# tigarcia/firedancer

Hardware: AMD Instinct MI355X
Metric: ed25519 verifies/sec at 1/8 GPUs; % INT32 VALU roofline; p99 batch latency (higher is better)
Workload: dtype int32

## Files before the change

### firedancer_amd/csrc/fd25519_dsm.h

```cpp
#pragma once
#include "fd25519_ge.h"
#include "fd_ed25519_hip_internal.h"

#define FD_ED25519_SUCCESS 0
#define FD_ED25519_ERR_SIG -1
#define FD_ED25519_ERR_PUBKEY -2
#define FD_ED25519_ERR_MSG -3


struct decoded_pt {
  fe x, y;
  bool fail;
  bool small;
};

FD_DEV void ge_decode(decoded_pt& d, const uint32_t (&s)[8], bool avx_rule) {
  const fe one = {{1, 0, 0, 0, 0, 0, 0, 0, 0, 0}};
  const fe cd = {FE_D}, sqrtm1 = {FE_SQRTM1};
  fe u, v, v3, x, vxx, t;
  fe_frombytes(d.y, s);
  const uint32_t sign = s[7] >> 31;
  fe_sq(u, d.y);
  fe_mul(v, u, cd);
  fe_sub(u, u, one);
// ... 103 lines not shown
  constexpr int W = SH / 32, B = SH % 32;
#pragma unroll
  for (int i = 4; i >= 0; i--) {
    const uint32_t hi = i - W >= 0 ? x[i - W] : 0u;
    const uint32_t lo = i - W - 1 >= 0 ? x[i - W - 1] : 0u;
    out[i] = B ? __builtin_amdgcn_alignbit(hi, lo, 32 - B) : hi;
  }
}

FD_DEV void shl160v(uint32_t (&out)[5], const uint32_t (&x)[5], int s) {
#pragma unroll
  for (int i = 4; i > 0; i--) out[i] = __builtin_amdgcn_alignbit(x[i], x[i - 1], 32 - s);
  out[0] = x[0] << s;
}

template <int BITS>
FD_DEV void recode160(uint32_t (&out)[5], const uint32_t (&x)[5]) {
  constexpr uint32_t M = (1u << BITS) - 1u;
  constexpr int PER = 32 / BITS;
  int carry = 0;
#pragma unroll
  for (int w = 0; w < 5; w++) {
    uint32_t packed = 0;
#pragma unroll
    for (int q = 0; q < PER; q++) {
      int e = (int)((x[w] >> (BITS * q)) & M) + carry;
      carry = (e + (1 << (BITS - 1))) >> BITS;
      e -= carry << BITS;
      packed |= ((uint32_t)e & M) << (BITS * q);
    }
    out[w] = packed;
  }
}

template <int BITS>
FD_DEV uint32_t pop160u(uint32_t (&d)[5]) {
  const uint32_t v = d[4] >> (32 - BITS);
#pragma unroll
  for (int w = 4; w > 0; w--) d[w] = __builtin_amdgcn_alignbit(d[w], d[w - 1], 32 - BITS);
  d[0] <<= BITS;
  return v;
}

template <int BITS>
FD_DEV int pop160(uint32_t (&d)[5]) {
  const int v = ((int32_t)d[4]) >> (32 - BITS);
#pragma unroll
  for (int w = 4; w > 0; w--) d[w] = __builtin_amdgcn_alignbit(d[w], d[w - 1], 32 - BITS);
  d[0] <<= BITS;
  return v;
}


FD_DEV void atab_store(int4* lane_tab, int e, const ge_cached& c) {
  int v[40];
#pragma unroll
  for (int i = 0; i < 10; i++) {
    v[i] = c.YplusX.v[i];
    v[10 + i] = c.YminusX.v[i];
    v[20 + i] = c.Z2.v[i];
    v[30 + i] = c.T2d.v[i];
  }
#pragma unroll
  for (int q = 0; q < 10; q++)
    lane_tab[e * 10 + q] = make_int4(v[4 * q], v[4 * q + 1], v[4 * q + 2], v[4 * q + 3]);
}

FD_DEV void atab_load(ge_cached& c, const int4* lane_tab, int e) {
  int v[40];
#pragma unroll
  for (int q = 0; q < 10; q++) {
    const int4 x = lane_tab[e * 10 + q];
    v[4 * q] = x.x; v[4 * q + 1] = x.y; v[4 * q + 2] = x.z; v[4 * q + 3] = x.w;
  }
#pragma unroll
  for (int i = 0; i < 10; i++) {
    c.YplusX.v[i] = v[i];
    c.YminusX.v[i] = v[10 + i];
    c.Z2.v[i] = v[20 + i];
    c.T2d.v[i] = v[30 + i];
  }
}

FD_DEV void btab_load(ge_precomp& b, const int4* s_btab, int e) {
  int v[32];
  const int4* src = s_btab + e * (FD_ED25519_BTAB_STRIDE / 4);
#pragma unroll
  for (int q = 0; q < 8; q++) {
    const int4 x = src[q];
    v[4 * q] = x.x; v[4 * q + 1] = x.y; v[4 * q + 2] = x.z; v[4 * q + 3] = x.w;
  }
#pragma unroll
  for (int i = 0; i < 10; i++) {
    b.yplusx.v[i] = v[i];
    b.yminusx.v[i] = v[10 + i];
    b.xy2d.v[i] = v[20 + i];
  }
}

FD_DEV void btab16_load(ge_precomp& b, const int4* g_btab, int e) {
  int v[32];
  const int4* src = g_btab + e * (FD_ED25519_BTAB16_STRIDE / 4);
#pragma unroll
  for (int q = 0; q < 8; q++) {
    const int4 x = src[q];
    v[4 * q] = x.x; v[4 * q + 1] = x.y; v[4 * q + 2] = x.z; v[4 * q + 3] = x.w;
  }
#pragma unroll
  for (int i = 0; i < 10; i++) {
    b.yplusx.v[i] = v[i];
    b.yminusx.v[i] = v[10 + i];
    b.xy2d.v[i] = v[20 + i];
  }
}


FD_DEV void ge_scalarmult_base(ge_p2& Q, const uint32_t (&s)[8], const int4* s_btab) {
  uint32_t sd[8];
  recode_radix256(sd, s);
  ge_p3 P;
  ge_p3_0(P);
  ge_p1p1 Rt;
#pragma clang loop unroll(disable)
  for (int j = 31; j >= 0; j--) {
    if (j != 31) {
#pragma clang loop unroll(disable)
      for (int dd = 0; dd < 8; dd++) {
        ge_p2_dbl(Rt, Q);
        if (dd < 7) ge_p1p1_to_p2(Q, Rt);
      }
      ge_p1p1_to_p3(P, Rt);
    }
    const int f = pop_digit<8>(sd);
    ge_precomp b;
    btab_load(b, s_btab, f < 0 ? -f : f);
    ge_precomp_cneg(b, f < 0);
    ge_madd(Rt, P, b);
    ge_p1p1_to_p2(Q, Rt);
  }
}

FD_DEV void ge_encode(uint32_t (&out)[8], const ge_p2& Q) {
  fe zi, x, y;
  fe_invert(zi, Q.Z);
  fe_mul(x, Q.X, zi);
  fe_mul(y, Q.Y, zi);
  uint32_t xb[8];
  fe_tobytes(xb, x);
  fe_tobytes(out, y);
  out[7] |= (xb[0] & 1u) << 31;
}
```

### firedancer_amd/csrc/fd25519_fe.h

```cpp
#pragma once
#include <hip/hip_runtime.h>
#include <stdint.h>

#define FD_DEV __device__ __forceinline__

struct fe { int32_t v[10]; };

#define FE_D      {-10913610, 13857413, -15372611, 6949391, 114729, -8787816, -6275908, -3247719, -18696448, -12055116}
#define FE_D2     {-21827239, -5839606, -30745221, 13898782, 229458, 15978800, -12551817, -6495438, 29715968, 9444199}
#define FE_DINV   {30013526, 3972531, -24787780, 12719051, 2979674, -4599962, -15693209, -3644061, 18959709, -16629253}
#define FE_SQRTM1 {-32595792, -7943725, 9377950, 3500415, 12389472, -272473, -25146209, -2005654, 326686, 11406482}
#define FE_BX     {-14297830, -7645148, 16144683, -16471763, 27570974, -2696100, -26142465, 8378389, 20764389, 8758491}
#define FE_BY     {-26843541, -6710886, 13421773, -13421773, 26843546, 6710886, -13421773, 13421773, -26843546, -6710886}

FD_DEV void fe_set_const(fe& h, const int32_t (&c)[10]) {
#pragma unroll
  for (int i = 0; i < 10; i++) h.v[i] = c[i];
}

FD_DEV void fe_0(fe& h) {
#pragma unroll
  for (int i = 0; i < 10; i++) h.v[i] = 0;
}

// ... 115 lines not shown
      const int k = i + j;
      const int m = (((i & 1) && (j & 1)) ? 2 : 1) * ((k >= 10) ? 19 : 1);
      const int32_t x = (i == j) ? f.v[i] : 2 * f.v[i];
      const int32_t y = m * f.v[j];
      if (i == 0) fe_mad_init(a[k], x, y, k);
      else fe_mad(a[k >= 10 ? k - 10 : k], x, y);
    }
  }
  fe_carry_wide(h, a);
}

FD_DEV void fe_sq2(fe& h, const fe& f) {
  int64_t a[10];
#pragma unroll
  for (int i = 0; i < 10; i++) {
#pragma unroll
    for (int j = i; j < 10; j++) {
      const int k = i + j;
      const int m = (((i & 1) && (j & 1)) ? 2 : 1) * ((k >= 10) ? 19 : 1);
      const int32_t x = (i == j) ? 2 * f.v[i] : 4 * f.v[i];
      const int32_t y = m * f.v[j];
      if (i == 0) fe_mad_init(a[k], x, y, k);
      else fe_mad(a[k >= 10 ? k - 10 : k], x, y);
    }
  }
  fe_carry_wide(h, a);
}

FD_DEV void fe_join_u(int32_t (&u)[10], int64_t c4, int64_t c9) {
  {
    const int64_t t = c4 + (int64_t)(uint32_t)u[5];
    u[5] = (int32_t)t & ((1 << 25) - 1);
    u[6] += (int32_t)(t >> 25);
  }
  {
    const int64_t t = c9 * 19 + (int64_t)(uint32_t)u[0];
    u[0] = (int32_t)t & ((1 << 26) - 1);
    u[1] += (int32_t)(t >> 26);
  }
}

FD_DEV void fe_launder_u(fe& h, int32_t (&u)[10]) {
#pragma unroll
  for (int i = 0; i < 10; i++) {
    asm("" : "+v"(u[i]));
    h.v[i] = u[i];
  }
}

FD_DEV void fe_mul19_u(fe& h, const fe& f, const fe& g, const fe& g19) {
  int32_t u[10];
  int64_t cA = 0, cB = 0;
#pragma unroll
  for (int s = 0; s < 5; s++) {
#pragma unroll
    for (int half = 0; half < 2; half++) {
      const int k = s + 5 * half;
      int64_t acc = half ? cB : cA;
#pragma unroll
      for (int n = 0; n < 10; n++) {
        const int i = n, j = (k - i + 10) % 10;
        const int32_t x = ((i & 1) && (j & 1)) ? 2 * f.v[i] : f.v[i];
        const int32_t y = (i + j >= 10) ? g19.v[j] : g.v[j];
        if (s == 0 && n == 0) acc = (int64_t)x * y;
        else acc += (int64_t)x * y;
#if FE_ASM_MAD
        FE_ACC_BARRIER_U(acc);
#endif
      }
      const int w = (k & 1) ? 25 : 26;
      u[k] = (int32_t)acc & ((1 << w) - 1);
      if (half) cB = acc >> w;
      else cA = acc >> w;
    }
  }
  fe_join_u(u, cA, cB);
  fe_launder_u(h, u);
}

FD_DEV void fe_mul_u(fe& h, const fe& f, const fe& g) {
  fe g19;
  fe_19(g19, g);
  fe_mul19_u(h, f, g, g19);
}

template <int S>
FD_DEV void fe_sqs_u(fe& h, const fe& f) {
  int32_t u[10];
  int64_t cA = 0, cB = 0;
#pragma unroll
  for (int s = 0; s < 5; s++) {
#pragma unroll
    for (int half = 0; half < 2; half++) {
      const int k = s + 5 * half;
      int64_t acc = half ? cB : cA;
      bool first = (s == 0);
#pragma unroll
      for (int i = 0; i < 10; i++) {
#pragma unroll
        for (int j = i; j < 10; j++) {
          if ((i + j) % 10 != k) continue;
          const int m = (((i & 1) && (j & 1)) ? 2 : 1) * ((i + j >= 10) ? 19 : 1);
          const int32_t x = (i == j) ? S * f.v[i] : 2 * S * f.v[i];
          const int32_t y = m * f.v[j];
          if (first) acc = (int64_t)x * y;
          else acc += (int64_t)x * y;
          first = false;
#if FE_ASM_MAD
          FE_ACC_BARRIER_U(acc);
#endif
        }
      }
      const int w = (k & 1) ? 25 : 26;
      u[k] = (int32_t)acc & ((1 << w) - 1);
      if (half) cB = acc >> w;
      else cA = acc >> w;
    }
  }
  fe_join_u(u, cA, cB);
  fe_launder_u(h, u);
}

FD_DEV void fe_sq_u(fe& h, const fe& f) { fe_sqs_u<1>(h, f); }
FD_DEV void fe_sq2_u(fe& h, const fe& f) { fe_sqs_u<2>(h, f); }

FD_DEV void fe_carry(fe& h, const fe& f) {
  int64_t a[10];
#pragma unroll
  for (int i = 0; i < 10; i++) a[i] = (int64_t)f.v[i] + FE_BIAS(i);
  fe_carry_wide(h, a);
}

FD_DEV void fe_frombytes(fe& h, const uint32_t (&w)[8]) {
  const uint32_t m26 = (1u << 26) - 1u, m25 = (1u << 25) - 1u;
  h.v[0] = (int32_t)(w[0] & m26);
  h.v[1] = (int32_t)(__builtin_amdgcn_alignbit(w[1], w[0], 26) & m25);
  h.v[2] = (int32_t)(__builtin_amdgcn_alignbit(w[2], w[1], 19) & m26);
  h.v[3] = (int32_t)(__builtin_amdgcn_alignbit(w[3], w[2], 13) & m25);
  h.v[4] = (int32_t)((w[3] >> 6) & m26);
  h.v[5] = (int32_t)(w[4] & m25);
  h.v[6] = (int32_t)(__builtin_amdgcn_alignbit(w[5], w[4], 25) & m26);
  h.v[7] = (int32_t)(__builtin_amdgcn_alignbit(w[6], w[5], 19) & m25);
  h.v[8] = (int32_t)(__builtin_amdgcn_alignbit(w[7], w[6], 12) & m26);
  h.v[9] = (int32_t)((w[7] >> 6) & m25);
}

FD_DEV void fe_carry(fe& h, const fe& f);
FD_DEV void fe_tobytes(uint32_t (&s)[8], const fe& f) {
  fe g;
  fe_carry(g, f);
  int32_t h[10];
#pragma unroll
  for (int i = 0; i < 10; i++) h[i] = g.v[i];
  int32_t q = (19 * h[9] + (1 << 24)) >> 25;
#pragma unroll
  for (int i = 0; i < 10; i++) q = (h[i] + q) >> ((i & 1) ? 25 : 26);
  h[0] += 19 * q;
  int32_t c;
#pragma unroll
  for (int i = 0; i < 9; i++) {
    const int sh = (i & 1) ? 25 : 26;
    c = h[i] >> sh;
    h[i + 1] += c;
    h[i] -= c * (1 << sh);
  }
  c = h[9] >> 25;
// ... 67 lines not shown
```

### firedancer_amd/csrc/fd25519_ge.h

```cpp
#pragma once
#include "fd25519_fe.h"

struct ge_p2 { fe X, Y, Z; };
struct ge_p3 { fe X, Y, Z, T; };
struct ge_p1p1 { fe X, Y, Z, T; };
struct ge_cached { fe YplusX, YminusX, Z2, T2d; };
struct ge_precomp { fe yplusx, yminusx, xy2d; };

FD_DEV void ge_p3_0(ge_p3& h) {
  fe_0(h.X); fe_1(h.Y); fe_1(h.Z); fe_0(h.T);
}


FD_DEV void ge_p1p1_to_p2(ge_p2& r, const ge_p1p1& p) {
  fe x19, z19;
  fe_19(x19, p.X);
  fe_19(z19, p.Z);
  fe_mul19_u(r.X, p.T, p.X, x19);
  fe_mul19_u(r.Y, p.Y, p.Z, z19);
  fe_mul19_u(r.Z, p.T, p.Z, z19);
}

template <bool UXYT, bool UZ>
FD_DEV void ge_p1p1_to_p3_t(ge_p3& r, const ge_p1p1& p) {
  fe x19, z19;
  fe_19(x19, p.X);
  fe_19(z19, p.Z);
  if (UXYT) {
    fe_mul19_u(r.X, p.T, p.X, x19);
    fe_mul19_u(r.T, p.Y, p.X, x19);
    fe_mul19_u(r.Y, p.Y, p.Z, z19);
  } else {
    fe_mul19(r.X, p.T, p.X, x19);
    fe_mul19(r.T, p.Y, p.X, x19);
    fe_mul19(r.Y, p.Y, p.Z, z19);
  }
  if (UZ) fe_mul19_u(r.Z, p.T, p.Z, z19);
  else fe_mul19(r.Z, p.T, p.Z, z19);
}

FD_DEV void ge_p1p1_to_p3(ge_p3& r, const ge_p1p1& p) { ge_p1p1_to_p3_t<false, false>(r, p); }
FD_DEV void ge_p1p1_to_p3_u(ge_p3& r, const ge_p1p1& p) { ge_p1p1_to_p3_t<true, true>(r, p); }
FD_DEV void ge_p1p1_to_p3_uxyt(ge_p3& r, const ge_p1p1& p) { ge_p1p1_to_p3_t<true, false>(r, p); }

FD_DEV void ge_p2_dbl(ge_p1p1& r, const ge_p2& p) {
  fe xx, yy, b, a, aa;
  fe_sq(xx, p.X);
  fe_sq_u(yy, p.Y);
  fe_sq2_u(b, p.Z);
  fe_sub(a, p.X, p.Y);
  fe_sq_u(aa, a);
  fe_add(r.Y, yy, xx);
  fe_sub(r.Z, yy, xx);
  fe_sub(r.X, r.Y, aa);
  fe_sub(r.T, b, r.Z);
}

FD_DEV void ge_p3_dbl(ge_p1p1& r, const ge_p3& p) {
  ge_p2 q;
  q.X = p.X; q.Y = p.Y; q.Z = p.Z;
  ge_p2_dbl(r, q);
}

#define FE_P_LIMBS {(1 << 26) - 19, (1 << 25) - 1, (1 << 26) - 1, (1 << 25) - 1, (1 << 26) - 1, \
                    (1 << 25) - 1, (1 << 26) - 1, (1 << 25) - 1, (1 << 26) - 1, (1 << 25) - 1}
template <bool UXY = false>
FD_DEV void ge_p3_to_cached(ge_cached& r, const ge_p3& p) {
  const fe d2 = {FE_D2};
  if (UXY) {
    const fe pl = {FE_P_LIMBS};
#pragma unroll
    for (int i = 0; i < 10; i++) r.YplusX.v[i] = p.Y.v[i] + p.X.v[i] - pl.v[i];
  } else {
    fe_add(r.YplusX, p.Y, p.X);
  }
  fe_sub(r.YminusX, p.Y, p.X);
  fe_add(r.Z2, p.Z, p.Z);
  fe_mul_u(r.T2d, p.T, d2);
}

template <bool NT = false>
FD_DEV void ge_add(ge_p1p1& r, const ge_p3& p, const ge_cached& q) {
  fe a, b, c, zz2;
  fe_add(a, p.Y, p.X);
  fe_sub(b, p.Y, p.X);
  fe_mul_u(a, a, q.YplusX);
  fe_mul_u(b, b, q.YminusX);
  fe_mul_u(zz2, p.Z, q.Z2);
  if (NT) fe_mul_u(c, q.T2d, p.T);
  else fe_mul(c, q.T2d, p.T);
  fe_sub(r.X, a, b);
  fe_add(r.Y, a, b);
  if (NT) {
    fe_sub(r.Z, zz2, c);
    fe_add(r.T, zz2, c);
  } else {
    fe_add(r.Z, zz2, c);
    fe_sub(r.T, zz2, c);
  }
}

FD_DEV void ge_madd(ge_p1p1& r, const ge_p3& p, const ge_precomp& q) {
  fe a, b, c, t0;
  fe_add(a, p.Y, p.X);
  fe_sub(b, p.Y, p.X);
  fe_mul_u(a, a, q.yplusx);
  fe_mul_u(b, b, q.yminusx);
  fe_mul(c, q.xy2d, p.T);
  fe_add(t0, p.Z, p.Z);
  fe_sub(r.X, a, b);
  fe_add(r.Y, a, b);
  fe_add(r.Z, t0, c);
  fe_sub(r.T, t0, c);
}

FD_DEV void ge_cached_cneg(ge_cached& q, bool neg) {
  fe t;
#pragma unroll
  for (int i = 0; i < 10; i++) {
    const int32_t a = q.YplusX.v[i], b = q.YminusX.v[i];
    q.YplusX.v[i] = neg ? b : a;
    q.YminusX.v[i] = neg ? a : b;
    t.v[i] = -q.T2d.v[i];
    q.T2d.v[i] = neg ? t.v[i] : q.T2d.v[i];
  }
}

FD_DEV void ge_precomp_cneg(ge_precomp& q, bool neg) {
#pragma unroll
  for (int i = 0; i < 10; i++) {
    const int32_t a = q.yplusx.v[i], b = q.yminusx.v[i];
    q.yplusx.v[i] = neg ? b : a;
    q.yminusx.v[i] = neg ? a : b;
    const int32_t t = q.xy2d.v[i];
    q.xy2d.v[i] = neg ? -t : t;
  }
}
```

### firedancer_amd/csrc/fd_ed25519_kernels.hip

```cpp
#include <hip/hip_runtime.h>
#include "fd25519_dsm.h"
#include "fd25519_ge4.h"
#include "fd25519_sc.h"
#include "fd_sha512_dev.h"
#define FD_HALF_FN __device__ static inline
#define FD_HALF_RCP(y) __builtin_amdgcn_rcp(y)
#define FD_HALF_RCPF(y) __builtin_amdgcn_rcpf(y)
#include "fd25519_half.h"



#define FD_PF_FAIL  1u
#define FD_PF_SMALL 2u
#define FD_HF_DNEG  1u
#define FD_HF_FULL  2u


FD_DEV uint32_t nblk_bucket(uint32_t sz) {
  const uint32_t b = (sz + 208u) >> 7;
  return b < (FD_ED25519_SORT_BUCKETS - 1) ? b : (FD_ED25519_SORT_BUCKETS - 1);
}

#define FD_SORT_PER_THREAD 16
#define FD_SORT_PER_BLOCK (256 * FD_SORT_PER_THREAD)
// ... 92 lines not shown
  uint32_t dig[16];
  if (p.digests) {
    const uint4* dg = reinterpret_cast<const uint4*>(p.digests + 64 * i);
#pragma unroll
    for (int q = 0; q < 4; q++) {
      const uint4 v = dg[q];
      dig[4 * q] = v.x; dig[4 * q + 1] = v.y; dig[4 * q + 2] = v.z; dig[4 * q + 3] = v.w;
    }
  } else {
    const uintptr_t mp = reinterpret_cast<uintptr_t>(p.msgs + p.msg_off[i]);
    sha_msg_src m;
    m.base = reinterpret_cast<const uint32_t*>(mp & ~(uintptr_t)3);
    m.shift = (uint32_t)(mp & 3);
    m.sz = p.msg_sz[i];
    sha512_ram(dig, r, a, m);
  }
  hash_finish(p, j, dig, S);
}

__global__ void __launch_bounds__(256, FD_ED25519_HASH_WAVES_PER_SIMD)
fd_ed25519_hash_kernel(fd_ed25519_verify_params_t p) {
  const uint64_t t = (uint64_t)blockIdx.x * blockDim.x + threadIdx.x;
  if (t >= p.n) return;
  hash_one(p, p.perm ? (uint64_t)p.perm[t] : t);
}

FD_DEV void decode_one(const fd_ed25519_verify_params_t& p, int which , uint64_t j) {
  const uint64_t i = p.base + j;
  uint32_t s[8];
  {
    const uint4* src = which ? reinterpret_cast<const uint4*>(p.sigs + 64 * i)
                             : reinterpret_cast<const uint4*>(p.pubs + 32 * i);
    const uint4 q0 = src[0], q1 = src[1];
    s[0] = q0.x; s[1] = q0.y; s[2] = q0.z; s[3] = q0.w; s[4] = q1.x; s[5] = q1.y; s[6] = q1.z; s[7] = q1.w;
  }
  decoded_pt d;
  ge_decode(d, s, !p.codes_portable);
  int32_t* dst = p.pts + (uint64_t)which * 20 * p.cap + j;
#pragma unroll
  for (int l = 0; l < 10; l++) {
    dst[(uint64_t)l * p.cap] = d.x.v[l];
    dst[(uint64_t)(10 + l) * p.cap] = d.y.v[l];
  }
  p.pflag[(uint64_t)which * p.cap + j] = (uint8_t)((d.fail ? FD_PF_FAIL : 0u) | (d.small ? FD_PF_SMALL : 0u));
}

__global__ void __launch_bounds__(256, FD_ED25519_DECODE_WAVES_PER_SIMD)
fd_ed25519_decode_kernel(fd_ed25519_verify_params_t p) {
  const uint64_t t = (uint64_t)blockIdx.x * blockDim.x + threadIdx.x;
  if (t >= 2 * p.n) return;
  const int which = t >= p.n;
  decode_one(p, which, which ? t - p.n : t);
}

FD_DEV void load_fe(fe& x, const int32_t* src, uint64_t cap) {
#pragma unroll
  for (int l = 0; l < 10; l++) x.v[l] = src[(uint64_t)l * cap];
}

FD_DEV void load_pt(fe& x, fe& y, const fd_ed25519_verify_params_t& p, int which, uint64_t j) {
  const int32_t* src = p.pts + (uint64_t)which * 20 * p.cap + j;
  load_fe(x, src, p.cap);
  load_fe(y, src + 10 * p.cap, p.cap);
}

#define FD_PENDING 1
FD_DEV int precheck(const fd_ed25519_verify_params_t& p, uint64_t j) {
  const uint32_t s_ok = p.sflag[j];
  const uint32_t af = p.pflag[j], rf = p.pflag[p.cap + j];
  if (!s_ok) return FD_ED25519_ERR_SIG;
  if (af & FD_PF_FAIL) return p.codes_portable ? FD_ED25519_ERR_PUBKEY : FD_ED25519_ERR_SIG;
  if (rf & FD_PF_FAIL) return FD_ED25519_ERR_SIG;
  if (af & FD_PF_SMALL) return FD_ED25519_ERR_PUBKEY;
  if (rf & FD_PF_SMALL) return FD_ED25519_ERR_SIG;
  return FD_PENDING;
}

template <bool NT>
FD_DEV void table_store(int4* tab, int e, ge_cached c) {
  if (NT) fe_neg(c.T2d, c.T2d);
  atab_store(tab, e, c);
}

__device__ const int4 fd_ident_cached[10] = {{1, 0, 0, 0}, {0, 0, 0, 0}, {0, 0, 1, 0}, {0, 0, 0, 0}, {0, 0, 0, 0},
                                             {2, 0, 0, 0}, {0, 0, 0, 0}, {0, 0, 0, 0}, {0, 0, 0, 0}, {0, 0, 0, 0}};

template <bool NT>
FD_DEV void table_build(int4* tab, const fe& x, const fe& y, bool negate) {
  ge_p3 P0;
  fe xn;
  fe_neg(xn, x);
  fe_select(P0.X, x, xn, negate);
  P0.Y = y;
  fe_1(P0.Z);
  fe_mul(P0.T, P0.X, y);
  ge_cached c1, c;
  c.YplusX = P0.Z; c.YminusX = P0.Z; fe_add(c.Z2, P0.Z, P0.Z); fe_0(c.T2d);
  atab_store(tab, 0, c);
  ge_p3_to_cached(c1, P0);
  table_store<NT>(tab, 1, c1);
  ge_precomp pre;
  pre.yplusx = c1.YplusX; pre.yminusx = c1.YminusX; pre.xy2d = c1.T2d;
  ge_p3 cur = P0;
  ge_p1p1 sum;
#pragma clang loop unroll(disable)
  for (int e = 2; e <= 8; e++) {
    ge_madd(sum, cur, pre);
    ge_p1p1_to_p3_uxyt(cur, sum);
    ge_p3_to_cached<true>(c, cur);
    table_store<NT>(tab, e, c);
  }
}

FD_DEV void table_add(ge_p1p1& Rt, const ge_p3& P, const int4* tab, int e) {
  ge_cached c;
  atab_load(c, tab, e < 0 ? -e : e);
  ge_cached_cneg(c, e < 0);
  ge_add(Rt, P, c);
}

FD_DEV void btab_add(ge_p1p1& Rt, const ge_p3& P, ge_precomp& b, int f) {
  ge_precomp_cneg(b, f < 0);
  ge_madd(Rt, P, b);
}


FD_DEV bool half_pair_ok(const uint32_t (&k)[8], const uint32_t (&c)[FD_HALF_TW], const uint32_t (&dm)[FD_HALF_TW],
                         int dneg, int dbits) {
  uint32_t x[16];
#pragma unroll
  for (int w = 0; w < 16; w++) x[w] = 0u;
#pragma unroll
  for (int a = 0; a < FD_HALF_TW; a++) {
    uint64_t carry = 0;
#pragma unroll
    for (int b = 0; b < 8; b++) {
      const uint64_t t = (uint64_t)dm[a] * k[b] + x[a + b] + carry;
      x[a + b] = (uint32_t)t;
      carry = t >> 32;
    }
    x[a + 8] = (uint32_t)carry;
  }
  const uint32_t n8l[8] = FD_HALF_N8L;
  uint32_t add[8];
  {
    uint64_t br = 0;
#pragma unroll
    for (int w = 0; w < 8; w++) {
      const uint32_t cv = w < FD_HALF_TW ? c[w] : 0u;
      const uint64_t t = (uint64_t)n8l[w] - cv - br;
      br = (t >> 63) & 1u;
      add[w] = dneg ? cv : (uint32_t)t;
    }
  }
  {
    uint64_t carry = 0;
#pragma unroll
    for (int w = 0; w < 15; w++) {
      const uint64_t t = (uint64_t)x[w] + (w < 8 ? add[w] : 0u) + carry;
      x[w] = (uint32_t)t;
      carry = t >> 32;
    }
  }
  const uint32_t low = x[0] & 7u;
#pragma unroll
  for (int w = 0; w < 15; w++) x[w] = __builtin_amdgcn_alignbit(x[w + 1], x[w], 3);
  x[15] >>= 3;
// ... 79 lines not shown
        const uint64_t t = (uint64_t)l[w] - sp[w] - br;
        br = (t >> 63) & 1u;
        sp[w] = nz ? (uint32_t)t : 0u;
      }
    }
  }
  uint32_t* hs = p.hs + j;
  const uint64_t c = p.cap;
  static_assert(FD_ED25519_BTABW_SHIFT == 144, "s_lo is words 0..3 and the low half of word 4");
#pragma unroll
  for (int w = 0; w < 5; w++) {
    hs[(uint64_t)w * c] = cw[w];
    hs[(uint64_t)(5 + w) * c] = dm[w];
    hs[(uint64_t)(10 + w) * c] = w < 4 ? sp[w] : (sp[4] & 0xffffu);
  }
#pragma unroll
  for (int w = 0; w < 4; w++)
    hs[(uint64_t)(15 + w) * c] = __builtin_amdgcn_alignbit(w + 5 < 8 ? sp[w + 5] : 0u, sp[w + 4], 16);
  p.hflag[j] = (uint8_t)((dneg ? FD_HF_DNEG : 0u) | (ok ? 0u : FD_HF_FULL));
  if (!ok && !p.small) {
    const uint32_t slot = atomicAdd(p.fix_cnt, 1u);
    p.fix_list[slot] = (uint32_t)j;
  }
}

__global__ void __launch_bounds__(256, FD_ED25519_SCALAR_WAVES_PER_SIMD)
fd_ed25519_scalar_kernel(fd_ed25519_verify_params_t p) {
  const uint64_t j = (uint64_t)blockIdx.x * blockDim.x + threadIdx.x;
  if (j >= p.n) return;
  scalar_one(p, j);
}

__global__ void __launch_bounds__(192) fd_ed25519_prep_kernel(fd_ed25519_verify_params_t p) {
  const uint32_t w = threadIdx.x >> 6;
  const uint64_t t = (uint64_t)blockIdx.x * 64u + (threadIdx.x & 63u);
  if (t >= p.n) return;
  if (w == 0) {
    const uint64_t j = p.perm ? (uint64_t)p.perm[t] : t;
    hash_one(p, j);
    scalar_one(p, j);
  } else {
    decode_one(p, (int)w - 1, t);
  }
}


FD_DEV void load_hs(uint32_t (&x)[5], const fd_ed25519_verify_params_t& p, int row, int words, uint64_t j) {
#pragma unroll
  for (int w = 0; w < 5; w++) x[w] = w < words ? p.hs[(uint64_t)(row + w) * p.cap + j] : 0u;
}

template <int BITS>
FD_DEV int wave_windows(const uint32_t (&d)[5]) {
  static_assert(BITS == 2 || BITS == 4, "2-bit or 4-bit windows");
  constexpr int W0 = 132 / BITS;
  int W = W0;
  const int wl = (fd_half_bitlen<5>(d) + BITS) >> (BITS / 2);
#pragma unroll
  for (int w = W0 + 1; w <= (FD_HALF_DBITS_MAX + BITS) / BITS; w++) W += __ballot(wl >= w) != 0ull;
  return W;
}

template <int BW>
struct fd_bw {
  static constexpr int STEP   = BW / 4;
  static constexpr int LO_N   = FD_ED25519_BTABW_SHIFT / BW;
  static constexpr int HI_N   = (253 - FD_ED25519_BTABW_SHIFT + BW - 1) / BW;
  static constexpr int LO_SHL = 160 - LO_N * BW;
  static constexpr int HI_SHL = 160 - HI_N * BW;
  static_assert(BW % 4 == 0, "base digits start at window boundaries");
  static_assert(LO_N * BW == FD_ED25519_BTABW_SHIFT, "s_lo digits cover bits 0..SHIFT-1");
  static_assert(HI_N * BW >= 253 - FD_ED25519_BTABW_SHIFT, "s_hi digits cover s' >> SHIFT");
  static_assert(STEP * (LO_N - 1) <= 32, "every base digit falls within the 33 windows");
  FD_DEV static bool lo_at(int it) { return it <= STEP * (LO_N - 1) && it % STEP == 0; }
  FD_DEV static bool hi_at(int it) { return it <= STEP * (HI_N - 1) && it % STEP == 0; }
};


FD_DEV void jtab_store(int4* tab, int slot, const ge_p3& P, bool neg) {
  ge_cached c;
  ge_p3_to_cached<true>(c, P);
  fe_neg(c.T2d, c.T2d);
  ge_cached_cneg(c, neg);
  atab_store(tab, slot, c);
}

FD_DEV void jtab_affine(ge_p3& P, const fd_ed25519_verify_params_t& p, int which, uint64_t j, bool negate) {
  fe x, xn;
  load_pt(x, P.Y, p, which, j);
  fe_neg(xn, x);
  fe_select(P.X, x, xn, negate);
  fe_1(P.Z);
  fe_mul(P.T, P.X, P.Y);
}

FD_DEV void jtab_step(int4* tab, int src, const ge_p3& q, int sp, int sm, bool mneg) {
  ge_cached e;
  atab_load(e, tab, src);
  fe qs, qd, m;
  fe_add(qs, q.Y, q.X);
  fe_sub(qd, q.Y, q.X);
  fe_mul(m, e.T2d, q.T);
#pragma clang loop unroll(disable)
  for (int h = sm < 0 ? 1 : 0; h < 2; h++) {
    const bool plus = h != 0;
    fe u, v, a, b, ms, mn;
    fe_select(u, qd, qs, plus);
    fe_select(v, qs, qd, plus);
    fe_mul_u(a, e.YplusX, u);
    fe_mul_u(b, e.YminusX, v);
    fe_neg(mn, m);
    fe_select(ms, mn, m, plus);
    ge_p1p1 sum;
    fe_sub(sum.X, a, b);
    fe_add(sum.Y, a, b);
    fe_sub(sum.Z, e.Z2, ms);
    fe_add(sum.T, e.Z2, ms);
    ge_p3 K;
    ge_p1p1_to_p3_uxyt(K, sum);
    jtab_store(tab, plus ? sp : sm, K, !plus && mneg);
  }
}

#define FD_JSLOT(a, r) (5 * (a) + (r) - 1)
FD_DEV void joint_table_build(int4* tab, const fd_ed25519_verify_params_t& p, uint64_t j, bool rneg) {
  ge_p3 P;
#pragma clang loop unroll(disable)
  for (int w = 0; w < 2; w++) {
    jtab_affine(P, p, w, j, w ? rneg : true);
    ge_cached c1;
    ge_p3_to_cached(c1, P);
    table_store<true>(tab, w ? FD_JSLOT(0, 1) : FD_JSLOT(1, 0), c1);
    ge_p1p1 sum;
    ge_p3_dbl(sum, P);
    ge_p3 D;
    ge_p1p1_to_p3_uxyt(D, sum);
    jtab_store(tab, w ? FD_JSLOT(0, 2) : FD_JSLOT(2, 0), D, false);
  }
#pragma clang loop unroll(disable)
  for (int st = 0; st < 4; st++) {
    const int src = st == 0 ? FD_JSLOT(0, 2) : st == 1 ? FD_JSLOT(1, 0) : st == 2 ? FD_JSLOT(2, 0) : FD_JSLOT(2, 1);
    const int sp = st == 0 ? FD_JSLOT(1, 2) : st == 1 ? FD_JSLOT(1, 1) : st == 2 ? FD_JSLOT(2, 1) : FD_JSLOT(2, 2);
    const int sm = st == 0 ? FD_JSLOT(1, -2) : st == 1 ? FD_JSLOT(1, -1) : st == 2 ? FD_JSLOT(2, -1) : -1;
    jtab_affine(P, p, st ? 1 : 0, j, st ? rneg : true);
    jtab_step(tab, src, P, sp, sm, st == 0);
  }
}

FD_DEV const int4* jtab_entry(const int4* tab, int a, int r) {
  const int slot = FD_JSLOT(a, r);
  return slot < 0 ? fd_ident_cached : tab + slot * 10;
}

template <int BW>
FD_DEV int dsm_half_one(const fd_ed25519_verify_params_t& p, uint64_t j, int4* tab) {
  int code = precheck(p, j);
  const uint32_t hf = p.hflag[j];
  joint_table_build(tab, p, j, !(hf & FD_HF_DNEG));
  uint32_t cd[5], dd[5], ld[5], hd[5];
  int W = 66;
  {
    uint32_t x[5], t[5];
    load_hs(x, p, 5, 5, j);
    const int wl = (fd_half_bitlen<5>(x) + 2) >> 1;
#pragma unroll
    for (int w = 67; w <= (FD_HALF_DBITS_MAX + 2) / 2; w++) W += __ballot(wl >= w) != 0ull;
    const int sh = 160 - 2 * W;
    shl160v(t, x, sh); recode160<2>(dd, t);
    load_hs(x, p, 0, 5, j);  shl160v(t, x, sh); recode160<2>(cd, t);
    load_hs(x, p, 10, 5, j); shl160<fd_bw<BW>::LO_SHL>(ld, x);
    load_hs(x, p, 15, 4, j); shl160<fd_bw<BW>::HI_SHL>(hd, x);
  }
  const int4* g_btab = reinterpret_cast<const int4*>(p.btab_lo);
  const int4* g_btab2 = reinterpret_cast<const int4*>(p.btab_hi);

  ge_p3 P;
  ge_p1p1 Rt;
  ge_p2 Q;
  {
    const int ea = pop160<2>(cd) & 3, er = pop160<2>(dd) & 3;
    ge_cached cj;
    atab_load(cj, jtab_entry(tab, ea, er), 0);
    fe t;
    fe_sub(t, cj.YplusX, cj.YminusX);
    fe_carry(Q.X, t);
    fe_add(t, cj.YplusX, cj.YminusX);
    fe_carry(Q.Y, t);
    Q.Z = cj.Z2;
  }
#pragma clang loop unroll(disable)
  for (int it = W - 2; it >= 0; it--) {
    const int ea = pop160<2>(cd), er = pop160<2>(dd);
    const bool sg = ea < 0 || (ea == 0 && er < 0);
    ge_cached cj;
    const bool blo = !(it & 1) && fd_bw<BW>::lo_at(it >> 1), bhi = !(it & 1) && fd_bw<BW>::hi_at(it >> 1);
    ge_precomp b1, b2;
    atab_load(cj, jtab_entry(tab, sg ? -ea : ea, sg ? -er : er), 0);
    if (blo) btab16_load(b1, g_btab, (int)pop160u<BW>(ld));
    if (bhi) btab16_load(b2, g_btab2, (int)pop160u<BW>(hd));
#pragma clang loop unroll(disable)
    for (int dbl = 0; dbl < 2; dbl++) {
      ge_p2_dbl(Rt, Q);
      if (dbl < 1) ge_p1p1_to_p2(Q, Rt);
    }
    ge_p1p1_to_p3_u(P, Rt);
    ge_cached_cneg(cj, sg);
    ge_add<true>(Rt, P, cj);
    if (blo) {
      ge_p1p1_to_p3_uxyt(P, Rt);
      ge_madd(Rt, P, b1);
    }
    if (bhi) {
      ge_p1p1_to_p3_uxyt(P, Rt);
      ge_madd(Rt, P, b2);
    }
    ge_p1p1_to_p2(Q, Rt);
  }
  fe t;
  fe_sub(t, Q.Y, Q.Z);
  const bool ident = fe_iszero(Q.X) && fe_iszero(t);
  if (code == FD_PENDING) code = ident ? FD_ED25519_SUCCESS : FD_ED25519_ERR_MSG;
  return code;
}

FD_DEV int dsm_full_core(const fd_ed25519_verify_params_t& p, uint64_t j, int4* tabA, int code, const fe& ax,
                         const fe& ay, const fe& rx, const fe& ry) {
  const uint64_t i = p.base + j;
  table_build<false>(tabA, ax, ay, true);
  uint32_t kd[8], sd[8];
  {
    uint32_t k[8], S[8];
#pragma unroll
    for (int w = 0; w < 8; w++) k[w] = p.k[(uint64_t)w * p.cap + j];
    const uint4* sg = reinterpret_cast<const uint4*>(p.sigs + 64 * i);
    const uint4 q2 = sg[2], q3 = sg[3];
    S[0] = q2.x; S[1] = q2.y; S[2] = q2.z; S[3] = q2.w; S[4] = q3.x; S[5] = q3.y; S[6] = q3.z; S[7] = q3.w;
    recode_radix16(kd, k);
    recode_radix65536(sd, S);
  }
  const int4* g_btab = reinterpret_cast<const int4*>(p.btab16);
  ge_p3 P;
  ge_p3_0(P);
  ge_p1p1 Rt;
  ge_p2 Q;
#pragma clang loop unroll(disable)
  for (int it = 63; it >= 0; it--) {
    const bool badd = (it & 3) == 0;
    int f = 0;
    ge_precomp b;
    if (badd) {
      f = pop_digit<16>(sd);
      btab16_load(b, g_btab, f < 0 ? -f : f);
    }
    if (it != 63) {
#pragma clang loop unroll(disable)
      for (int dbl = 0; dbl < 4; dbl++) {
        ge_p2_dbl(Rt, Q);
        if (dbl < 3) ge_p1p1_to_p2(Q, Rt);
      }
      ge_p1p1_to_p3_u(P, Rt);
    }
    table_add(Rt, P, tabA, pop_digit<4>(kd));
    if (badd) {
      ge_p1p1_to_p3_uxyt(P, Rt);
      btab_add(Rt, P, b, f);
    }
    ge_p1p1_to_p2(Q, Rt);
  }
  fe t1, t2;
  fe_mul(t1, rx, Q.Z);
  fe_sub(t1, t1, Q.X);
  fe_mul(t2, ry, Q.Z);
  fe_sub(t2, t2, Q.Y);
  const bool eq = fe_iszero(t1) && fe_iszero(t2);
  if (code != FD_PENDING) return code;
  return eq ? FD_ED25519_SUCCESS : FD_ED25519_ERR_MSG;
}

FD_DEV int dsm_full_one(const fd_ed25519_verify_params_t& p, uint64_t j, int4* tabA) {
  fe ax, ay, rx, ry;
  load_pt(ax, ay, p, 0, j);
  load_pt(rx, ry, p, 1, j);
  return dsm_full_core(p, j, tabA, precheck(p, j), ax, ay, rx, ry);
}

template <int BW>
__global__ void __launch_bounds__(FD_ED25519_VERIFY_BLOCK, FD_ED25519_DSM_WAVES_PER_SIMD)
fd_ed25519_dsm_kernel(fd_ed25519_verify_params_t p) {
  const uint32_t lane = threadIdx.x & 63u;
  const uint64_t wave = ((uint64_t)blockIdx.x * blockDim.x + threadIdx.x) >> 6;
  int4* tabA = reinterpret_cast<int4*>(static_cast<char*>(p.atab) + wave * FD_ED25519_ATAB_BYTES_PER_WAVE) +
               lane * (2 * FD_ED25519_ATAB_STRIDE * 10);
  if (p.small) {
    const uint64_t stride = (uint64_t)gridDim.x * blockDim.x;
    for (uint64_t t = (uint64_t)blockIdx.x * blockDim.x + threadIdx.x; t < p.n; t += stride)
      if (p.hflag[t] & FD_HF_FULL) p.out[p.base + t] = (int8_t)dsm_full_one(p, t, tabA);
    return;
  }
  const uint64_t nfix = *p.fix_cnt;
  const uint64_t head = (nfix + 63u) & ~(uint64_t)63u;
  const uint64_t total = head + p.n;
  for (;;) {
    uint32_t b = 0u;
    if (lane == 0u) b = atomicAdd(p.work_ctr, 64u);
    b = (uint32_t)__builtin_amdgcn_readfirstlane((int)__shfl((int)b, 0));
    if ((uint64_t)b >= total) break;
    const uint64_t t = (uint64_t)b + lane;
    if (t < nfix) {
      const uint64_t j = p.fix_list[t];
      p.out[p.base + j] = (int8_t)dsm_full_one(p, j, tabA);
    } else if (t >= head && t < total) {
      const uint64_t j = t - head;
      if (!(p.hflag[j] & FD_HF_FULL)) p.out[p.base + j] = (int8_t)dsm_half_one<BW>(p, j, tabA);
    }
  }
}


FD_DEV void tab4_store(int4* tab, int e, const fe& c) {
  int4* d = tab + 3 * e;
  d[0] = make_int4(c.v[0], c.v[1], c.v[2], c.v[3]);
  d[1] = make_int4(c.v[4], c.v[5], c.v[6], c.v[7]);
  d[2] = make_int4(c.v[8], c.v[9], 0, 0);
}

FD_DEV void tab4_load(fe& c, const int4* tab, int e) {
  const int4* s = tab + 3 * e;
  const int4 a = s[0], b = s[1], d = s[2];
  c.v[0] = a.x; c.v[1] = a.y; c.v[2] = a.z; c.v[3] = a.w;
  c.v[4] = b.x; c.v[5] = b.y; c.v[6] = b.z; c.v[7] = b.w;
  c.v[8] = d.x; c.v[9] = d.y;
}

FD_DEV void btab4_load(fe& c, const int32_t* g_btab, int e, const qmask_t& m) {
  const int off = m.l0 ? 10 : (m.l1 ? 0 : 20);
  const int2* s = reinterpret_cast<const int2*>(g_btab + (size_t)e * FD_ED25519_BTAB16_STRIDE + off);
#pragma unroll
  for (int q = 0; q < 5; q++) {
    const int2 x = s[q];
    c.v[2 * q] = x.x;
    c.v[2 * q + 1] = x.y;
  }
#pragma unroll
  for (int i = 0; i < 10; i++) c.v[i] = m.l3 ? (i == 0 ? 2 : 0) : c.v[i];
}

FD_DEV void table4_build(int4* tab, const fe& x, const fe& y, bool negate, const qmask_t& m) {
  fe xs, xy, p0, c1, c, r, cur;
#pragma unroll
  for (int i = 0; i < 10; i++) xs.v[i] = negate ? -x.v[i] : x.v[i];
  fe_mul(xy, xs, y);
#pragma unroll
  for (int i = 0; i < 10; i++) {
    p0.v[i] = m.l0 ? xs.v[i] : (m.l1 ? y.v[i] : (m.l2 ? (i == 0 ? 1 : 0) : xy.v[i]));
    c.v[i] = i == 0 ? (m.l2 ? 0 : (m.l3 ? 2 : 1)) : 0;
  }
  tab4_store(tab, 0, c);
  ge4_to_qc(c1, p0, m);
  tab4_store(tab, 1, c1);
  cur = p0;
#pragma clang loop unroll(disable)
  for (int e = 2; e <= 8; e++) {
    ge4_add(r, cur, c1, m);
    ge4_to_p3(cur, r);
    ge4_to_qc(c, cur, m);
    tab4_store(tab, e, c);
  }
}

FD_DEV void ge4_dbl4(fe& P, const qmask_t& m) {
  fe Rt;
#pragma clang loop unroll(disable)
  for (int dbl = 0; dbl < 4; dbl++) {
    ge4_dbl(Rt, P, m);
    ge4_to_p3(P, Rt);
  }
}

FD_DEV void ge4_add_signed(fe& P, const fe& c, bool neg, const qmask_t& m) {
  fe Rt;
  ge4_cneg(P, m.l03, neg);
  ge4_add(Rt, P, c, m);
  ge4_cneg(Rt, m.l0, neg);
  ge4_to_p3(P, Rt);
}

FD_DEV void quad_finish(const fd_ed25519_verify_params_t& p, uint64_t j, const fe& P, int code, bool store) {
  fe y1, z1, t;
  fe_qp<FD_QP(1, 1, 1, 1)>(y1, P);
  fe_qp<FD_QP(2, 2, 2, 2)>(z1, P);
  fe_sub(t, y1, z1);
  const bool ident = fe_iszero(P) && fe_iszero(t);
  if (code == FD_PENDING) code = ident ? FD_ED25519_SUCCESS : FD_ED25519_ERR_MSG;
  if (store) p.out[p.base + j] = (int8_t)code;
}

// ... 788 lines not shown
```

Before: 108.8 million.

## Restructure joint table build and half-DSM loop with fused conditional negation

Changes the joint-table entry layout so negation becomes a swap of YplusX/YminusX halves at load time, with T2d negated inside the multiply via a sign-scaled operand, which removes the separate cached-negate pass. The table build caches the affine input points in shared memory instead of recomputing them, shares the Z product between the plus and minus entries, and computes K.Z once. The main loop extracts digits with sbfe from a word that shifts only every 16 iterations, instead of a 5-word shift per step. The identity-cached entry is changed to match the new layout. Shared memory use rises by 60 words per thread, which may lower occupancy.

```diff
diff --git a/firedancer_amd/csrc/fd25519_dsm.h b/firedancer_amd/csrc/fd25519_dsm.h
--- a/firedancer_amd/csrc/fd25519_dsm.h
+++ b/firedancer_amd/csrc/fd25519_dsm.h
@@ -209,6 +209,49 @@
   }
 }
 
+FD_DEV void jent_store(int4* ent, const ge_cached& c) {
+  const int32_t* p = c.YplusX.v;
+  const int32_t* m = c.YminusX.v;
+  ent[0] = make_int4(p[0], p[1], p[2], p[3]);
+  ent[1] = make_int4(p[4], p[5], p[6], p[7]);
+  ent[2] = make_int4(m[0], m[1], m[2], m[3]);
+  ent[3] = make_int4(m[4], m[5], m[6], m[7]);
+  ent[4] = make_int4(p[8], p[9], m[8], m[9]);
+  int v[20];
+#pragma unroll
+  for (int i = 0; i < 10; i++) {
+    v[i] = c.Z2.v[i];
+    v[10 + i] = c.T2d.v[i];
+  }
+#pragma unroll
+  for (int q = 0; q < 5; q++) ent[5 + q] = make_int4(v[4 * q], v[4 * q + 1], v[4 * q + 2], v[4 * q + 3]);
+}
+
+FD_DEV void jent_load(ge_cached& c, const int4* ent, bool neg) {
+  const int4* hp = ent + (neg ? 2 : 0);
+  const int4* hm = ent + (neg ? 0 : 2);
+  const int4 p0 = hp[0], p1 = hp[1], m0 = hm[0], m1 = hm[1], t = ent[4];
+  c.YplusX.v[0] = p0.x; c.YplusX.v[1] = p0.y; c.YplusX.v[2] = p0.z; c.YplusX.v[3] = p0.w;
+  c.YplusX.v[4] = p1.x; c.YplusX.v[5] = p1.y; c.YplusX.v[6] = p1.z; c.YplusX.v[7] = p1.w;
+  c.YminusX.v[0] = m0.x; c.YminusX.v[1] = m0.y; c.YminusX.v[2] = m0.z; c.YminusX.v[3] = m0.w;
+  c.YminusX.v[4] = m1.x; c.YminusX.v[5] = m1.y; c.YminusX.v[6] = m1.z; c.YminusX.v[7] = m1.w;
+  c.YplusX.v[8] = neg ? t.z : t.x;
+  c.YplusX.v[9] = neg ? t.w : t.y;
+  c.YminusX.v[8] = neg ? t.x : t.z;
+  c.YminusX.v[9] = neg ? t.y : t.w;
+  int v[20];
+#pragma unroll
+  for (int q = 0; q < 5; q++) {
+    const int4 x = ent[5 + q];
+    v[4 * q] = x.x; v[4 * q + 1] = x.y; v[4 * q + 2] = x.z; v[4 * q + 3] = x.w;
+  }
+#pragma unroll
+  for (int i = 0; i < 10; i++) {
+    c.Z2.v[i] = v[i];
+    c.T2d.v[i] = v[10 + i];
+  }
+}
+
 FD_DEV void btab_load(ge_precomp& b, const int4* s_btab, int e) {
   int v[32];
   const int4* src = s_btab + e * (FD_ED25519_BTAB_STRIDE / 4);
diff --git a/firedancer_amd/csrc/fd25519_fe.h b/firedancer_amd/csrc/fd25519_fe.h
--- a/firedancer_amd/csrc/fd25519_fe.h
+++ b/firedancer_amd/csrc/fd25519_fe.h
@@ -221,6 +221,20 @@
   fe g19;
   fe_19(g19, g);
   fe_mul19_u(h, f, g, g19);
+}
+
+FD_DEV void fe_mul_u_cneg(fe& h, const fe& f, const fe& g, bool neg) {
+  int32_t s = neg ? -1 : 1, s19 = neg ? -19 : 19;
+  asm("" : "+v"(s));
+  asm("" : "+v"(s19));
+  fe gs, gs19;
+  gs19.v[0] = 0;
+#pragma unroll
+  for (int j = 0; j < 10; j++) {
+    gs.v[j] = s * g.v[j];
+    if (j) gs19.v[j] = s19 * g.v[j];
+  }
+  fe_mul19_u(h, f, gs, gs19);
 }
 
 template <int S>
diff --git a/firedancer_amd/csrc/fd25519_ge.h b/firedancer_amd/csrc/fd25519_ge.h
--- a/firedancer_amd/csrc/fd25519_ge.h
+++ b/firedancer_amd/csrc/fd25519_ge.h
@@ -100,6 +100,20 @@
   }
 }
 
+FD_DEV void ge_add_nt_cneg(ge_p1p1& r, const ge_p3& p, const ge_cached& q, bool neg) {
+  fe a, b, c, zz2;
+  fe_add(a, p.Y, p.X);
+  fe_sub(b, p.Y, p.X);
+  fe_mul_u(a, a, q.YplusX);
+  fe_mul_u(b, b, q.YminusX);
+  fe_mul_u(zz2, p.Z, q.Z2);
+  fe_mul_u_cneg(c, q.T2d, p.T, neg);
+  fe_sub(r.X, a, b);
+  fe_add(r.Y, a, b);
+  fe_sub(r.Z, zz2, c);
+  fe_add(r.T, zz2, c);
+}
+
 FD_DEV void ge_madd(ge_p1p1& r, const ge_p3& p, const ge_precomp& q) {
   fe a, b, c, t0;
   fe_add(a, p.Y, p.X);
diff --git a/firedancer_amd/csrc/fd_ed25519_kernels.hip b/firedancer_amd/csrc/fd_ed25519_kernels.hip
--- a/firedancer_amd/csrc/fd_ed25519_kernels.hip
+++ b/firedancer_amd/csrc/fd_ed25519_kernels.hip
@@ -198,7 +198,7 @@
   atab_store(tab, e, c);
 }
 
-__device__ const int4 fd_ident_cached[10] = {{1, 0, 0, 0}, {0, 0, 0, 0}, {0, 0, 1, 0}, {0, 0, 0, 0}, {0, 0, 0, 0},
+__device__ const int4 fd_ident_cached[10] = {{1, 0, 0, 0}, {0, 0, 0, 0}, {1, 0, 0, 0}, {0, 0, 0, 0}, {0, 0, 0, 0},
                                              {2, 0, 0, 0}, {0, 0, 0, 0}, {0, 0, 0, 0}, {0, 0, 0, 0}, {0, 0, 0, 0}};
 
 template <bool NT>
@@ -444,7 +444,7 @@
   ge_p3_to_cached<true>(c, P);
   fe_neg(c.T2d, c.T2d);
   ge_cached_cneg(c, neg);
-  atab_store(tab, slot, c);
+  jent_store(tab + slot * 10, c);
 }
 
 FD_DEV void jtab_affine(ge_p3& P, const fd_ed25519_verify_params_t& p, int which, uint64_t j, bool negate) {
@@ -456,43 +456,77 @@
   fe_mul(P.T, P.X, P.Y);
 }
 
+#define FD_JKEEP_WORDS 60
+FD_DEV void jtab_keep(int32_t* keep, int which, const ge_p3& P) {
+#pragma unroll
+  for (int i = 0; i < 10; i++) {
+    keep[(30 * which + i) * FD_ED25519_VERIFY_BLOCK] = P.X.v[i];
+    keep[(30 * which + 10 + i) * FD_ED25519_VERIFY_BLOCK] = P.Y.v[i];
+    keep[(30 * which + 20 + i) * FD_ED25519_VERIFY_BLOCK] = P.T.v[i];
+  }
+}
+
+FD_DEV void jtab_kept(ge_p3& P, const int32_t* keep, int which) {
+#pragma unroll
+  for (int i = 0; i < 10; i++) {
+    P.X.v[i] = keep[(30 * which + i) * FD_ED25519_VERIFY_BLOCK];
+    P.Y.v[i] = keep[(30 * which + 10 + i) * FD_ED25519_VERIFY_BLOCK];
+    P.T.v[i] = keep[(30 * which + 20 + i) * FD_ED25519_VERIFY_BLOCK];
+  }
+  fe_1(P.Z);
+}
+
 FD_DEV void jtab_step(int4* tab, int src, const ge_p3& q, int sp, int sm, bool mneg) {
   ge_cached e;
-  atab_load(e, tab, src);
+  jent_load(e, tab + src * 10, false);
   fe qs, qd, m;
   fe_add(qs, q.Y, q.X);
   fe_sub(qd, q.Y, q.X);
   fe_mul(m, e.T2d, q.T);
+  fe zs, zt, kz;
+  fe_sub(zs, e.Z2, m);
+  fe_add(zt, e.Z2, m);
+  {
+    fe z19;
+    fe_19(z19, zs);
+    fe_mul19(kz, zt, zs, z19);
+  }
 #pragma clang loop unroll(disable)
   for (int h = sm < 0 ? 1 : 0; h < 2; h++) {
     const bool plus = h != 0;
-    fe u, v, a, b, ms, mn;
+    fe u, v, a, b;
     fe_select(u, qd, qs, plus);
     fe_select(v, qs, qd, plus);
     fe_mul_u(a, e.YplusX, u);
     fe_mul_u(b, e.YminusX, v);
-    fe_neg(mn, m);
-    fe_select(ms, mn, m, plus);
     ge_p1p1 sum;
     fe_sub(sum.X, a, b);
     fe_add(sum.Y, a, b);
-    fe_sub(sum.Z, e.Z2, ms);
-    fe_add(sum.T, e.Z2, ms);
+    fe_select(sum.Z, zt, zs, plus);
+    fe_select(sum.T, zs, zt, plus);
     ge_p3 K;
-    ge_p1p1_to_p3_uxyt(K, sum);
+    fe x19, z19;
+    fe_19(x19, sum.X);
+    fe_19(z19, sum.Z);
+    fe_mul19_u(K.X, sum.T, sum.X, x19);
+    fe_mul19_u(K.T, sum.Y, sum.X, x19);
+    fe_mul19_u(K.Y, sum.Y, sum.Z, z19);
+    K.Z = kz;
     jtab_store(tab, plus ? sp : sm, K, !plus && mneg);
   }
 }
 
 #define FD_JSLOT(a, r) (5 * (a) + (r) - 1)
-FD_DEV void joint_table_build(int4* tab, const fd_ed25519_verify_params_t& p, uint64_t j, bool rneg) {
+FD_DEV void joint_table_build(int4* tab, const fd_ed25519_verify_params_t& p, uint64_t j, bool rneg, int32_t* keep) {
   ge_p3 P;
 #pragma clang loop unroll(disable)
   for (int w = 0; w < 2; w++) {
     jtab_affine(P, p, w, j, w ? rneg : true);
+    jtab_keep(keep, w, P);
     ge_cached c1;
     ge_p3_to_cached(c1, P);
-    table_store<true>(tab, w ? FD_JSLOT(0, 1) : FD_JSLOT(1, 0), c1);
+    fe_neg(c1.T2d, c1.T2d);
+    jent_store(tab + (w ? FD_JSLOT(0, 1) : FD_JSLOT(1, 0)) * 10, c1);
     ge_p1p1 sum;
     ge_p3_dbl(sum, P);
     ge_p3 D;
@@ -504,7 +538,7 @@
     const int src = st == 0 ? FD_JSLOT(0, 2) : st == 1 ? FD_JSLOT(1, 0) : st == 2 ? FD_JSLOT(2, 0) : FD_JSLOT(2, 1);
     const int sp = st == 0 ? FD_JSLOT(1, 2) : st == 1 ? FD_JSLOT(1, 1) : st == 2 ? FD_JSLOT(2, 1) : FD_JSLOT(2, 2);
     const int sm = st == 0 ? FD_JSLOT(1, -2) : st == 1 ? FD_JSLOT(1, -1) : st == 2 ? FD_JSLOT(2, -1) : -1;
-    jtab_affine(P, p, st ? 1 : 0, j, st ? rneg : true);
+    jtab_kept(P, keep, st ? 1 : 0);
     jtab_step(tab, src, P, sp, sm, st == 0);
   }
 }
@@ -515,21 +549,20 @@
 }
 
 template <int BW>
-FD_DEV int dsm_half_one(const fd_ed25519_verify_params_t& p, uint64_t j, int4* tab) {
+FD_DEV int dsm_half_one(const fd_ed25519_verify_params_t& p, uint64_t j, int4* tab, int32_t* keep) {
   int code = precheck(p, j);
   const uint32_t hf = p.hflag[j];
-  joint_table_build(tab, p, j, !(hf & FD_HF_DNEG));
+  joint_table_build(tab, p, j, !(hf & FD_HF_DNEG), keep);
   uint32_t cd[5], dd[5], ld[5], hd[5];
   int W = 66;
   {
-    uint32_t x[5], t[5];
+    uint32_t x[5];
     load_hs(x, p, 5, 5, j);
     const int wl = (fd_half_bitlen<5>(x) + 2) >> 1;
 #pragma unroll
     for (int w = 67; w <= (FD_HALF_DBITS_MAX + 2) / 2; w++) W += __ballot(wl >= w) != 0ull;
-    const int sh = 160 - 2 * W;
-    shl160v(t, x, sh); recode160<2>(dd, t);
-    load_hs(x, p, 0, 5, j);  shl160v(t, x, sh); recode160<2>(cd, t);
+    recode160<2>(dd, x);
+    load_hs(x, p, 0, 5, j);  recode160<2>(cd, x);
     load_hs(x, p, 10, 5, j); shl160<fd_bw<BW>::LO_SHL>(ld, x);
     load_hs(x, p, 15, 4, j); shl160<fd_bw<BW>::HI_SHL>(hd, x);
   }
@@ -540,9 +573,10 @@
   ge_p1p1 Rt;
   ge_p2 Q;
   {
-    const int ea = pop160<2>(cd) & 3, er = pop160<2>(dd) & 3;
+    const int tsh = 2 * ((W - 1) & 15);
+    const int ea = (int)(cd[4] >> tsh) & 3, er = (int)(dd[4] >> tsh) & 3;
     ge_cached cj;
-    atab_load(cj, jtab_entry(tab, ea, er), 0);
+    jent_load(cj, jtab_entry(tab, ea, er), false);
     fe t;
     fe_sub(t, cj.YplusX, cj.YminusX);
     fe_carry(Q.X, t);
@@ -552,12 +586,19 @@
   }
 #pragma clang loop unroll(disable)
   for (int it = W - 2; it >= 0; it--) {
-    const int ea = pop160<2>(cd), er = pop160<2>(dd);
+    if ((it & 15) == 15) {
+#pragma unroll
+      for (int w = 4; w > 0; w--) {
+        cd[w] = cd[w - 1];
+        dd[w] = dd[w - 1];
+      }
+    }
+    const int ea = __builtin_amdgcn_sbfe((int)cd[4], 2 * (it & 15), 2), er = __builtin_amdgcn_sbfe((int)dd[4], 2 * (it & 15), 2);
     const bool sg = ea < 0 || (ea == 0 && er < 0);
     ge_cached cj;
     const bool blo = !(it & 1) && fd_bw<BW>::lo_at(it >> 1), bhi = !(it & 1) && fd_bw<BW>::hi_at(it >> 1);
     ge_precomp b1, b2;
-    atab_load(cj, jtab_entry(tab, sg ? -ea : ea, sg ? -er : er), 0);
+    jent_load(cj, jtab_entry(tab, sg ? -ea : ea, sg ? -er : er), sg);
     if (blo) btab16_load(b1, g_btab, (int)pop160u<BW>(ld));
     if (bhi) btab16_load(b2, g_btab2, (int)pop160u<BW>(hd));
 #pragma clang loop unroll(disable)
@@ -566,8 +607,7 @@
       if (dbl < 1) ge_p1p1_to_p2(Q, Rt);
     }
     ge_p1p1_to_p3_u(P, Rt);
-    ge_cached_cneg(cj, sg);
-    ge_add<true>(Rt, P, cj);
+    ge_add_nt_cneg(Rt, P, cj, sg);
     if (blo) {
       ge_p1p1_to_p3_uxyt(P, Rt);
       ge_madd(Rt, P, b1);
@@ -653,6 +693,8 @@
   const uint64_t wave = ((uint64_t)blockIdx.x * blockDim.x + threadIdx.x) >> 6;
   int4* tabA = reinterpret_cast<int4*>(static_cast<char*>(p.atab) + wave * FD_ED25519_ATAB_BYTES_PER_WAVE) +
                lane * (2 * FD_ED25519_ATAB_STRIDE * 10);
+  __shared__ int32_t s_keep[FD_JKEEP_WORDS * FD_ED25519_VERIFY_BLOCK];
+  int32_t* keep = s_keep + threadIdx.x;
   if (p.small) {
     const uint64_t stride = (uint64_t)gridDim.x * blockDim.x;
     for (uint64_t t = (uint64_t)blockIdx.x * blockDim.x + threadIdx.x; t < p.n; t += stride)
@@ -673,7 +715,7 @@
       p.out[p.base + j] = (int8_t)dsm_full_one(p, j, tabA);
     } else if (t >= head && t < total) {
       const uint64_t j = t - head;
-      if (!(p.hflag[j] & FD_HF_FULL)) p.out[p.base + j] = (int8_t)dsm_half_one<BW>(p, j, tabA);
+      if (!(p.hflag[j] & FD_HF_FULL)) p.out[p.base + j] = (int8_t)dsm_half_one<BW>(p, j, tabA, keep);
     }
   }
 }
```

Result: no change. 109.8 million, median of 6 (+0.8%).
